# iacopo97/Multimodal-SAM-Adapter

Measured on AMD Instinct MI355X. Metric: images/sec encoder fwd @1024x1024 RGB+LiDAR ViT-L, higher is better.
Workload: dtype split-operand MFMA: fp16 hi + e5m2 cross terms (h8c / h8 planes, ViT / interaction / up-conv GEMMs) fp16 hi/lo pairs x3 (TwinConvNeXt: f3 planes) and bf16 hi/lo x3 (neck, head); attention blocks with the rel-pos terms fused: every contraction on one fp16 MFMA (q, k, v, P rounded to fp16) in the bloc

## Files before the change

include/mmsa.h:

```cpp
#ifndef MMSA_H
#define MMSA_H
#include <stddef.h>
#include <stdint.h>
#ifdef __cplusplus
extern "C" {
#endif

#ifdef MMSA_BUILDING_LIBRARY
typedef hipStream_t mmsa_stream_t;
#else
typedef void* mmsa_stream_t;
#endif

#include "mmsa_version.h"
int mmsa_version(void);
const char* mmsa_last_error(void);

int mmsa_debug_poison_lds(unsigned pattern, mmsa_stream_t stream);
int mmsa_event_create(void** ev);
int mmsa_event_record(void* ev, mmsa_stream_t stream);
int mmsa_event_elapsed_ms(void* start, void* stop, float* ms);
int mmsa_event_destroy(void* ev);

enum { MMSA_ACT_NONE = 0, MMSA_ACT_GELU = 1, MMSA_ACT_RELU = 2, MMSA_ACT_RELU6 = 3, MMSA_ACT_HSWISH = 4, MMSA_ACT_SIGMOID = 5 };
// ... 41 lines not shown
                            long strideW2, const float* b1, const float* b2, const float* gamma, float* x, long ldx, long strideX,
                            int M, int C, int batch, int max_grid, int fmt,
                            float* clamp_max , mmsa_stream_t stream);

int mmsa_split_planes(const float* src, long ld, int rows, int cols, int cols_pad, uint16_t* planes, int kind,
                      float* clamp_max , mmsa_stream_t stream);

int mmsa_attention(const float* qkv, long ldq, const float* qkv_bias, const float* rp, float* out, long ldo, int B,
                   int H, int W, int heads, int head_dim, int window_size, float scale, mmsa_stream_t stream);
int mmsa_attention_planes(const uint16_t* qkv_planes, long ldq, const uint16_t* bias_planes, const float* rp,
                          uint16_t* out_planes, long ldo, int B, int H, int W, int heads, int head_dim,
                          int window_size, float scale, int out_fmt ,
                          int v_fmt ,
                          float* max_abs_logit , mmsa_stream_t stream);

int mmsa_relpos_bias(const float* qkv, long ldq, const float* Rh, const float* Rw, float* rp, int B, int H, int W,
                     int heads, int head_dim, int window_size, mmsa_stream_t stream);
int mmsa_relpos_bias_planes(const uint16_t* qkv_planes, long ldq, const float* Rh, const float* Rw,
                            float* rp, int B, int H, int W, int heads, int head_dim, int window_size, mmsa_stream_t stream);

int mmsa_layernorm_rows(const float* x, long ldx, const float* w, const float* b, float eps, float* y, long ldy,
                        float* y2, long ldy2, uint16_t* y_planes, long ldp ,
                        int rows, int C, int map_mode, int map_H, int map_W, int group_rows, long w_gstride, long y_gcol,
                        int y_wrap, int plane_fmt , float* clamp_max ,
                        mmsa_stream_t stream);

int mmsa_colstats(const float* x, long ldx, long strideB, const float* wrow, int B, int HW, int C, double* out,
                  int out_is_zero , mmsa_stream_t stream);

int mmsa_ffrm_finalize(const double* stats, int B, int HW, int C, float mean_w, float mean_b, const float* Wc,
                       const float* gn_w, const float* gn_b, float* mean_o, float* rstd_o, float* mult_o,
                       float* scratch , mmsa_stream_t stream);
int mmsa_lnhw_apply(const float* x, long ldx, const float* mean, const float* rstd, const float* mult, const float* w,
                    const float* bias, float* y, long ldy, int B, int HW, int C, mmsa_stream_t stream);

int mmsa_dwconv_nhwc(const float* x, long ldx, long xstrideB, const float* w, const float* bias, float* y, long ldy,
                     long ystrideB, uint16_t* y_planes, long ldp, long pstrideB , int planes_fmt ,
                     int B, int H, int W, int C, int k, int act,
                     int imgs_per_group ,
                     float* rowstats ,
                     float* clamp_max , mmsa_stream_t stream);
int mmsa_gconv_nhwc(const float* x, long ldx, const float* w, const float* bias, float* y, long ldy, int B, int H,
                    int W, int G, int cin_g, int cout_g, int k, int act, mmsa_stream_t stream);
int mmsa_gfe_qkv_conv(const float* x, long ldx, const float* w, float* y, long ldy, int B, int H, int W, int G, int cin_g, int cout_g,
                      int* covered, mmsa_stream_t stream);
int mmsa_dwpair_gate(const float* x, long ldx, const float* w, float* y, long ldy, uint16_t* y_planes, long ldp, int B, int H,
                     int W, int C, mmsa_stream_t stream);
int mmsa_im2col_nchw(const float* x, int B, int Ctot, int c0, int Cin, int H, int W, int p, float* out, int Kpad,
                     mmsa_stream_t stream);

long mmsa_gram_tn_scratch_bytes(int B, int P, int c);
int mmsa_gram_tn(const float* X, long ldx, const float* Y, long ldy, long strideB, double* G , int B, int P, int c,
                 int nblk, void* scratch, long scratch_bytes, mmsa_stream_t stream);
int mmsa_chanattn_build(const double* G, const double* sq, long sq_strideB, const double* sk, long sk_strideB,
                        const float* temp, const float* Wp, uint16_t* planes , int B, int c, int cpad,
                        int heads, mmsa_stream_t stream);
int mmsa_gffm_build(const double* E, uint16_t* x_planes, uint16_t* y_planes , int B, int c,
                    int cpad, mmsa_stream_t stream);
int mmsa_gelu_gate(const float* x, long ldx, float* y, long ldy, long rows, int C, mmsa_stream_t stream);
int mmsa_pool_hw(const float* z, long ldz, float* out, long ldo, int B, int H, int W, int C, mmsa_stream_t stream);
int mmsa_ca_apply(const float* z, long ldz, const float* att, long lda, float* out, long ldo,
                  uint16_t* out_planes, long ldp , int B, int H, int W, int C, mmsa_stream_t stream);

int mmsa_tail_fuse(const float* cmap, long ldc, long cstrideB, const float* xtok, long ldx, const float* bn_scale,
                   const float* bn_shift, float* out, uint16_t* out_planes , long ldp,
                   int B, int Hc, int Wc, int Hx, int Wx, int C, mmsa_stream_t stream);

int mmsa_global_attention_planes(const uint16_t* qkv_planes, long ldq, const uint16_t* bias_planes, const uint16_t* relpos_planes,
                                 uint16_t* out_planes, long ldo, int B, int H, int W, int heads, int head_dim, float scale,
                                 int out_fmt , int v_fmt ,
                                 float* max_abs_logit , mmsa_stream_t stream);

int mmsa_window_attention_planes(const uint16_t* qkv_planes, long ldq, const uint16_t* bias_planes,
                                 const uint16_t* relpos_planes, const uint16_t* selector, uint16_t* out_planes, long ldo, int B, int H, int W,
                                 int heads, int head_dim, int window_size, float scale, int out_fmt ,
                                 int v_fmt , float* max_abs_logit , mmsa_stream_t stream);

int mmsa_nchw_to_planes(const float* src, long strideB, uint16_t* planes, long ldp, int B, int C, long HW,
                        mmsa_stream_t stream);
int mmsa_head_fuse(const float* z0, const float* z1, int H1, int W1, const float* z2, int H2, int W2, const float* z3,
                   int H3, int W3, long ld, const float* bn_scale, const float* bn_shift, uint16_t* planes, long ldp,
                   float* out32, long ldo, int B, int H, int W, int C, int act, mmsa_stream_t stream);
int mmsa_tokens_to_nchw(const float* src, long ld, float* dst, int B, long HW, int C, mmsa_stream_t stream);

int mmsa_bilinear_accum_nchw(const float* src, long src_strideB, int B, int C, int hs, int ws, float* dst, int Hd, int Wd, int y0, int x0,
                             int hc, int wc, float* count, int accumulate, mmsa_stream_t stream);
int mmsa_div_count_nchw(float* x, const float* count, int B, int C, long HW, mmsa_stream_t stream);
int mmsa_argmax_nchw(const float* x, unsigned char* out, int B, int C, long HW, mmsa_stream_t stream);
int mmsa_crop_batch_nchw(const float* src, int B, int C, int H, int W, const int* windows, int n, float* dst, int hc, int wc,
                         mmsa_stream_t stream);
int mmsa_slide_argmax(const float* logits, int n, int C, int hs, int ws, const int* windows, unsigned char* out, int B, int H, int W,
                      int hc, int wc, int* uncovered, mmsa_stream_t stream);
int mmsa_slide_argmax_resized(const float* logits, int n, int C, int hs, int ws, const int* windows, unsigned char* out, int B, int H, int W,
                              int hc, int wc, int Hd, int Wd, int Hcut, int Wcut, int* uncovered, mmsa_stream_t stream);

int mmsa_softmax_flip_accum_nchw(const float* logits, float* acc, int B, int C, int H, int W, int flip, int accumulate, int finish_div, mmsa_stream_t stream);
int mmsa_aug_argmax(const float* const* logits, const int* views, int A, int C, const int* windows, const int* windows_host, int total,
                    unsigned char* out, int B, int Ho, int Wo, int* uncovered, mmsa_stream_t stream);

int mmsa_argmax_max_nchw(const float* x, unsigned char* out, float* maxval, int B, int C, long HW, mmsa_stream_t stream);
int mmsa_slide_argmax_conf(const float* logits, int n, int C, int hs, int ws, const int* windows, unsigned char* out, float* conf, int B, int H, int W,
                           int hc, int wc, int* uncovered, mmsa_stream_t stream);
int mmsa_slide_argmax_resized_conf(const float* logits, int n, int C, int hs, int ws, const int* windows, unsigned char* out, float* conf, int B, int H,
                                   int W, int hc, int wc, int Hd, int Wd, int Hcut, int Wcut, int* uncovered, mmsa_stream_t stream);
int mmsa_aug_argmax_conf(const float* const* logits, const int* views, int A, int C, const int* windows, const int* windows_host, int total,
                         unsigned char* out, float* conf, int B, int Ho, int Wo, int* uncovered, mmsa_stream_t stream);

enum { MMSA_PRE_U8 = 0, MMSA_PRE_F32 = 1 };
int mmsa_preprocess_nhwc(const void* src0, int dtype0, const void* src1, int dtype1, int B, int Hs, int Ws, const float* mean,
                         const float* sinv, const int* div255, const int* swap, const float* pad_val, float* dst, int H, int W,
                         mmsa_stream_t stream);
int mmsa_preprocess_crops(const void* src0, int dtype0, const void* src1, int dtype1, int B, int Hs, int Ws, const float* mean,
                          const float* sinv, const int* div255, const int* swap, const float* pad_val, int H, int W, const int* windows,
                          int n, float* dst, int hc, int wc, mmsa_stream_t stream);
int mmsa_preprocess_resize_nhwc(const void* src0, int dtype0, const void* src1, int dtype1, int B, int Hs, int Ws, const float* mean,
                                const float* sinv, const int* div255, const int* swap, const float* pad_val, float* dst, int H, int W,
                                int Hr, int Wr, const int* xofs, const void* xcoef, const int* yofs, const void* ycoef, int fixed_point,
                                mmsa_stream_t stream);
int mmsa_preprocess_resize_crops(const void* src0, int dtype0, const void* src1, int dtype1, int B, int Hs, int Ws, const float* mean,
                                 const float* sinv, const int* div255, const int* swap, const float* pad_val, int H, int W, const int* windows,
                                 int n, float* dst, int hc, int wc, int Hr, int Wr, const int* xofs, const void* xcoef, const int* yofs,
                                 const void* ycoef, int fixed_point, mmsa_stream_t stream);

int mmsa_eval_confusion_u8(const unsigned char* pred, const unsigned char* label, int B, int H, int W, int Hl, int Wl, const unsigned char* lut,
                           int C, const int* ymap, const int* xmap, const int* slots, int n_slots, int64_t* counts, mmsa_stream_t stream);
int mmsa_slide_argmax_eval(const float* logits, int n, int C, int hs, int ws, const int* windows, unsigned char* out, int B, int H, int W,
                           int hc, int wc, int* uncovered, const unsigned char* label, int Hl, int Wl, const unsigned char* lut, const int* ymap,
                           const int* xmap, const int* slots, int n_slots, int64_t* counts, mmsa_stream_t stream);

int mmsa_eval_calibration(const unsigned char* pred, const float* conf, const unsigned char* label, int B, int H, int W, int Hl, int Wl,
                          const unsigned char* lut, int C, const int* ymap, const int* xmap, const int* slots, int n_slots, int bins, int64_t* cal,
                          mmsa_stream_t stream);

int mmsa_eval_selective(const unsigned char* pred, const float* conf, const unsigned char* label, int B, int H, int W, int Hl, int Wl,
                        const unsigned char* lut, int C, const int* ymap, const int* xmap, const int* slots, int n_slots, int bins, int64_t* counts,
                        mmsa_stream_t stream);
int mmsa_abstain_u8(const unsigned char* pred, const float* conf, long n, int bins, int min_bin, unsigned char* out, mmsa_stream_t stream);

int mmsa_slide_argmax_conf_t(const float* logits, int n, int C, int hs, int ws, const int* windows, unsigned char* out, float* conf, int B, int H, int W,
                             int hc, int wc, int* uncovered, float inv_temperature, mmsa_stream_t stream);
int mmsa_slide_argmax_resized_conf_t(const float* logits, int n, int C, int hs, int ws, const int* windows, unsigned char* out, float* conf, int B, int H,
                                     int W, int hc, int wc, int Hd, int Wd, int Hcut, int Wcut, int* uncovered, float inv_temperature, mmsa_stream_t stream);
int mmsa_softmax_flip_accum_nchw_t(const float* logits, float* acc, int B, int C, int H, int W, int flip, int accumulate, int finish_div,
                                   float inv_temperature, mmsa_stream_t stream);
int mmsa_temperature_sweep_nchw(const float* logits, const unsigned char* label, int B, int C, int H, int W, int Hl, int Wl, const unsigned char* lut,
                                const int* ymap, const int* xmap, const int* slots, int n_slots, const float* inv_temperatures, int J, int bins,
                                int64_t* sweep, mmsa_stream_t stream);

int mmsa_argmax_score_nchw(const float* prob, unsigned char* out, float* score, int B, int C, int H, int W, int kind, float inv_log_c, mmsa_stream_t stream);
int mmsa_slide_argmax_score(const float* logits, int n, int C, int hs, int ws, const int* windows, unsigned char* out, float* score, int B, int H, int W,
                            int hc, int wc, int* uncovered, int kind, float inv_temperature, float inv_log_c, mmsa_stream_t stream);
int mmsa_slide_argmax_resized_score(const float* logits, int n, int C, int hs, int ws, const int* windows, unsigned char* out, float* score, int B, int H,
                                    int W, int hc, int wc, int Hd, int Wd, int Hcut, int Wcut, int* uncovered, int kind, float inv_temperature,
                                    float inv_log_c, mmsa_stream_t stream);

int mmsa_slide_argmax_topk(const float* logits, int n, int C, int hs, int ws, const int* windows, unsigned char* classes, float* probs, int B, int H, int W,
                           int hc, int wc, int* uncovered, int K, float inv_temperature, mmsa_stream_t stream);
int mmsa_argmax_topk_nchw(const float* prob, const unsigned char* first, unsigned char* classes, float* probs, int B, int C, int H, int W, int K,
                          mmsa_stream_t stream);
int mmsa_eval_topk_u8(const unsigned char* classes, int K, const unsigned char* label, int B, int H, int W, int Hl, int Wl, const unsigned char* lut, int C,
                      const int* ymap, const int* xmap, const int* slots, int n_slots, int64_t* counts, mmsa_stream_t stream);

int mmsa_eval_boundary_u8(const unsigned char* pred, const unsigned char* label, int B, int H, int W, int Hl, int Wl, const unsigned char* lut, int C,
                          const int* ymap, const int* xmap, const int* slots, int n_slots, int radius, int border, int64_t* counts, mmsa_stream_t stream);

int mmsa_boundary_distance_u8(const unsigned char* src, int B, int Hs, int Ws, const unsigned char* lut, const int* ymap, const int* xmap, int H, int W,
// ... 76 lines not shown
```

multimodal-sam-adapter_amd/mmsa/head.py:

```python
import torch
import torch.nn as nn

from . import lib
from . import ops
from .params import Node, _attach


class SegformerHead(nn.Module):
    def __init__(self, interpolate_mode="bilinear", in_channels=None, channels=None, *, num_classes=None, dropout_ratio=0.1,
                 conv_cfg=None, norm_cfg=None, act_cfg=dict(type="ReLU"), in_index=-1, input_transform="multiple_select",
                 loss_decode=None, ignore_index=255, sampler=None, align_corners=False, init_cfg=None, **kwargs):
        super().__init__()
        if in_channels is None or channels is None or num_classes is None:
            raise TypeError("SegformerHead: in_channels, channels and num_classes are required")
        if not isinstance(in_channels, (list, tuple)) or not isinstance(in_index, (list, tuple)) or len(in_channels) != len(in_index):
            raise AssertionError("SegformerHead: in_channels and in_index must be lists of equal length")
        if not 1 <= len(in_channels) <= 4:
            raise NotImplementedError("mmsa SegformerHead: 1..4 input maps")
        if interpolate_mode != "bilinear" or align_corners:
            raise NotImplementedError("mmsa SegformerHead: only interpolate_mode='bilinear', align_corners=False (the reference configs)")
        if norm_cfg is None or norm_cfg.get("type") not in ("BN", "SyncBN"):
            raise NotImplementedError("mmsa SegformerHead: norm_cfg must be BN / SyncBN (eval: running-statistics affine)")
        if act_cfg is None or act_cfg.get("type") != "ReLU":
            raise NotImplementedError("mmsa SegformerHead: act_cfg must be ReLU")
        if channels % 8:
            raise NotImplementedError("mmsa SegformerHead: channels must be a multiple of 8")
        self.in_channels, self.in_index, self.channels = list(in_channels), list(in_index), channels
        self.num_classes, self.dropout_ratio, self.align_corners = num_classes, dropout_ratio, align_corners
        self.interpolate_mode, self.ignore_index, self.norm_cfg, self.act_cfg = interpolate_mode, ignore_index, norm_cfg, act_cfg
        n = len(in_channels)
        g = torch.Generator().manual_seed(0)

        def conv_w(co, ci):
            return torch.randn(co, ci, 1, 1, generator=g) * (2.0 / ci) ** 0.5

        def bn(prefix):
            _attach(self, prefix + ".weight", torch.ones(channels))
            _attach(self, prefix + ".bias", torch.zeros(channels))
            _attach(self, prefix + ".running_mean", torch.zeros(channels), buffer=True)
            _attach(self, prefix + ".running_var", torch.ones(channels), buffer=True)
            _attach(self, prefix + ".num_batches_tracked", torch.zeros((), dtype=torch.long), buffer=True)

        _attach(self, "conv_seg.weight", torch.randn(num_classes, channels, 1, 1, generator=g) * 0.01)
        _attach(self, "conv_seg.bias", torch.zeros(num_classes))
        self.add_module("convs", Node())
        for i, ci in enumerate(in_channels):
            _attach(self, f"convs.{i}.conv.weight", conv_w(channels, ci))
            bn(f"convs.{i}.bn")
        _attach(self, "fusion_conv.conv.weight", conv_w(channels, channels * n))
        bn("fusion_conv.bn")
        self._packed = None
        self._bufs = {}
        self.register_load_state_dict_post_hook(lambda m, _: m.invalidate())
        self.eval()

    def invalidate(self):
        self._packed = None

    def train(self, mode=True):
        if mode:
            raise NotImplementedError("mmsa: the MI355X decode head implements the inference forward path only")
        return super().train(False)

    def init_weights(self):
        pass

    def forward_test(self, inputs, img_metas=None, test_cfg=None):
        return self.forward(inputs)

    def forward_train(self, inputs, img_metas, gt_semantic_seg, train_cfg):
        raise NotImplementedError("mmsa: the MI355X decode head implements the inference forward path only (no losses)")

    @torch.no_grad()
    def _pack(self, dev):
        sd = {k: v.detach().to(dev, torch.float32) for k, v in self.state_dict().items() if v.dtype.is_floating_point}
        ch, n = self.channels, len(self.in_channels)

        def bn_affine(p):
            s = sd[p + ".weight"] / torch.sqrt(sd[p + ".running_var"] + 1e-5)
            return s.contiguous(), (sd[p + ".bias"] - sd[p + ".running_mean"] * s).contiguous()

        pk = {"branch": []}
        wf = sd["fusion_conv.conv.weight"].reshape(ch, ch * n)
        for i, ci in enumerate(self.in_channels):
            s, t = bn_affine(f"convs.{i}.bn")
            w = sd[f"convs.{i}.conv.weight"].reshape(ch, ci) * s[:, None]
            pk["branch"].append(dict(w=ops.split_planes(w.contiguous()), shift=t,
                                     wf=ops.split_planes(wf[:, ch * i:ch * (i + 1)].contiguous())))
        pk["fs"], pk["ft"] = bn_affine("fusion_conv.bn")
        ncp = ops.pad32(self.num_classes)
        wc = torch.zeros(ncp, ch, device=dev)
        wc[:self.num_classes] = sd["conv_seg.weight"].reshape(self.num_classes, ch)
        bc = torch.zeros(ncp, device=dev)
        bc[:self.num_classes] = sd["conv_seg.bias"]
        pk["wc"], pk["bc"], pk["ncp"] = ops.split_planes(wc), bc, ncp
        return pk

    def _buf(self, name, shape, dtype=torch.float32, dev=None):
        name = getattr(self, "buf_tag", "") + name
        t = self._bufs.get(name)
        if t is None or tuple(t.shape) != tuple(shape) or t.device != dev:
            t = torch.zeros(shape, dtype=dtype, device=dev)
            self._bufs[name] = t
        return t

    def _planes(self, name, rows, cols, dev):
        kp = ops.pad32(cols)
        return ops.Planes(self._buf(name, (rows, 2 * kp), torch.int16, dev), rows, cols, kp)

    @torch.no_grad()
    def forward(self, inputs, out=None):
        x0 = inputs[self.in_index[0]]
        if not x0.is_cuda:
            raise RuntimeError("mmsa SegformerHead: inputs must live on the GPU (there is no CPU path)")
        with torch.cuda.device(x0.device):
            return self._forward(inputs, out)

    def _forward(self, inputs, out=None):
        xs = [inputs[i] for i in self.in_index]
        x0 = xs[0]
        dev = x0.device
        if self._packed is None or self._packed["wc"].p.device != dev:
            self._packed = self._pack(dev)
        pk = self._packed
        B, _, H, W = x0.shape
        ch = self.channels
        zs = []
        for i, (x, ci) in enumerate(zip(xs, self.in_channels)):
            if x.dtype != torch.float32 or x.dim() != 4 or x.shape[0] != B or x.shape[1] != ci:
                raise RuntimeError(f"mmsa SegformerHead: input {i} must be fp32 [B={B}, {ci}, h, w], got {tuple(x.shape)} {x.dtype}")
            x = x.contiguous()
            h, w = x.shape[2:]
            rows = B * h * w
            xp = getattr(inputs[self.in_index[i]], "_mmsa_planes", None)
            if not isinstance(xp, ops.Planes) or xp.n != rows or xp.k != ci or xp.p.device != dev or not xp.live():
                xp = self._planes(f"x{i}", rows, ci, dev)
                lib.call("mmsa_nchw_to_planes", x.data_ptr(), ci * h * w, xp.p.data_ptr(), 2 * xp.kpad, B, ci, h * w, ops._stream())
            br = pk["branch"][i]
            yp = self._planes(f"y{i}", rows, ch, dev)
            ops.gemm(xp, br["w"], bias=br["shift"], act="relu", out_planes=yp)
            z = self._buf(f"z{i}", (rows, ch), dev=dev)
            ops.gemm(yp, br["wf"], z)
            zs.append((z, h, w))
        fp = self._planes("fused", B * H * W, ch, dev)
        lv = zs[1:] + [(None, 0, 0)] * (4 - len(zs))
        lib.call("mmsa_head_fuse", zs[0][0].data_ptr(),
                 lv[0][0].data_ptr() if lv[0][0] is not None else None, lv[0][1], lv[0][2],
                 lv[1][0].data_ptr() if lv[1][0] is not None else None, lv[1][1], lv[1][2],
                 lv[2][0].data_ptr() if lv[2][0] is not None else None, lv[2][1], lv[2][2],
                 ch, pk["fs"].data_ptr(), pk["ft"].data_ptr(), fp.p.data_ptr(), 2 * fp.kpad, None, 0, B, H, W, ch, ops.ACT["relu"],
                 ops._stream())
        lt = self._buf("logit_tokens", (B * H * W, pk["ncp"]), dev=dev)
        ops.gemm(fp, pk["wc"], lt, bias=pk["bc"])
        if out is None:
            out = torch.empty(B, self.num_classes, H, W, device=dev)
        elif (tuple(out.shape) != (B, self.num_classes, H, W) or out.dtype != torch.float32 or out.device != dev or not out.is_contiguous()):
            raise RuntimeError(f"mmsa SegformerHead: out must be a contiguous fp32 [{B}, {self.num_classes}, {H}, {W}] tensor on {dev}")
        lib.call("mmsa_tokens_to_nchw", lt.data_ptr(), pk["ncp"], out.data_ptr(), B, H * W, self.num_classes, ops._stream())
        return out
```

multimodal-sam-adapter_amd/mmsa/lib.py:

```python
import ctypes
import os
from ctypes import c_char_p, c_double, c_float, c_int, c_long, c_void_p, POINTER

_HERE = os.path.dirname(os.path.abspath(__file__))
LIB_PATH = os.environ.get("MMSA_LIB") or os.path.join(_HERE, "libmmsa_hip.so")

if not os.path.exists(LIB_PATH):
    raise RuntimeError(
        f"{LIB_PATH} not found: the MI355X HIP library is required (no CPU/PyTorch fallback exists). "
        "Build it with: python multimodal-sam-adapter_amd/build.py")

import torch

_lib = ctypes.CDLL(LIB_PATH)

P = c_void_p
I = c_int
L = c_long
F = c_float

_PAINT_TAIL = [P, I, P, I, I, I, I, I, P, P, I, I, c_double, c_double, c_double, c_double, P, P]
SIGNATURES = {
    "mmsa_version": [],
    "mmsa_last_error": [],
    "mmsa_debug_poison_lds": [ctypes.c_uint, P],
    "mmsa_event_create": [POINTER(c_void_p)],
    "mmsa_event_record": [P, P],
    "mmsa_event_elapsed_ms": [P, P, POINTER(c_float)],
    "mmsa_event_destroy": [P],
    "mmsa_ms_deform_attn_forward": [P, P, P, P, P, P, I, I, I, I, I, I, I, I, I, P],
    "mmsa_ms_deform_attn_backward": [P, P, P, P, P, P, P, P, P, I, I, I, I, I, I, I, I, I, P],
    "mmsa_msda_fused": [P, P, P, P, L, P, P, L, P, L, I, I, I, I, I, I, I, I, P, P],
    "mmsa_msda_fused_planes": [P, L, I, P, P, P, L, P, P, L, P, L, I, I, I, I, I, I, I, I, P, P],
    "mmsa_gemm_split3": [P, P, L, L, P, L, P, L, P, P, L, L, I, F, P, L, L, P, L, L, I, I, I, I, I, F, I, I, I, I, I, I, I, P, P, P, I, P, P],
    "mmsa_convnext_mlp_fused": [P, L, L, P, L, P, L, P, P, P, P, L, L, I, I, I, I, I, P, P],
    "mmsa_rowstats_finalize": [P, I, I, I, F, P, P],
    "mmsa_zero_bytes": [P, ctypes.c_size_t, P],
    "mmsa_split_planes": [P, L, I, I, I, P, I, P, P],
    "mmsa_attention": [P, L, P, P, P, L, I, I, I, I, I, I, F, P],
    "mmsa_attention_planes": [P, L, P, P, P, L, I, I, I, I, I, I, F, I, I, P, P],
    "mmsa_relpos_bias": [P, L, P, P, P, I, I, I, I, I, I, P],
    "mmsa_relpos_bias_planes": [P, L, P, P, P, I, I, I, I, I, I, P],
    "mmsa_layernorm_rows": [P, L, P, P, F, P, L, P, L, P, L, I, I, I, I, I, I, L, L, I, I, P, P],
    "mmsa_colstats": [P, L, L, P, I, I, I, P, I, P],
    "mmsa_ffrm_finalize": [P, I, I, I, F, F, P, P, P, P, P, P, P, P],
    "mmsa_lnhw_apply": [P, L, P, P, P, P, P, P, L, I, I, I, P],
    "mmsa_dwconv_nhwc": [P, L, L, P, P, P, L, L, P, L, L, I, I, I, I, I, I, I, I, P, P, P],
    "mmsa_dwpair_gate": [P, L, P, P, L, P, L, I, I, I, I, P],
    "mmsa_gconv_nhwc": [P, L, P, P, P, L, I, I, I, I, I, I, I, I, P],
    "mmsa_gfe_qkv_conv": [P, L, P, P, L, I, I, I, I, I, I, POINTER(c_int), P],
    "mmsa_im2col_nchw": [P, I, I, I, I, I, I, I, P, I, P],
    "mmsa_gram_tn": [P, L, P, L, L, P, I, I, I, I, P, L, P],
    "mmsa_gram_tn_scratch_bytes": [I, I, I],
    "mmsa_chanattn_build": [P, P, L, P, L, P, P, P, I, I, I, I, P],
    "mmsa_gffm_build": [P, P, P, I, I, I, P],
    "mmsa_gelu_gate": [P, L, P, L, L, I, P],
    "mmsa_pool_hw": [P, L, P, L, I, I, I, I, P],
    "mmsa_ca_apply": [P, L, P, L, P, L, P, L, I, I, I, I, P],
    "mmsa_tail_fuse": [P, L, L, P, L, P, P, P, P, L, I, I, I, I, I, I, P],
    "mmsa_global_attention_planes": [P, L, P, P, P, L, I, I, I, I, I, F, I, I, P, P],
    "mmsa_window_attention_planes": [P, L, P, P, P, P, L, I, I, I, I, I, I, F, I, I, P, P],
    "mmsa_nchw_to_planes": [P, L, P, L, I, I, L, P],
    "mmsa_head_fuse": [P, P, I, I, P, I, I, P, I, I, L, P, P, P, L, P, L, I, I, I, I, I, P],
    "mmsa_tokens_to_nchw": [P, L, P, I, L, I, P],
    "mmsa_bilinear_accum_nchw": [P, L, I, I, I, I, P, I, I, I, I, I, I, P, I, P],
    "mmsa_div_count_nchw": [P, P, I, I, L, P],
    "mmsa_argmax_nchw": [P, P, I, I, L, P],
    "mmsa_crop_batch_nchw": [P, I, I, I, I, P, I, P, I, I, P],
    "mmsa_slide_argmax": [P, I, I, I, I, P, P, I, I, I, I, I, P, P],
    "mmsa_slide_argmax_resized": [P, I, I, I, I, P, P, I, I, I, I, I, I, I, I, I, P, P],
    "mmsa_softmax_flip_accum_nchw": [P, P, I, I, I, I, I, I, I, P],
    "mmsa_aug_argmax": [P, P, I, I, P, P, I, P, I, I, I, P, P],
    "mmsa_argmax_max_nchw": [P, P, P, I, I, L, P],
    "mmsa_slide_argmax_conf": [P, I, I, I, I, P, P, P, I, I, I, I, I, P, P],
    "mmsa_slide_argmax_resized_conf": [P, I, I, I, I, P, P, P, I, I, I, I, I, I, I, I, I, P, P],
    "mmsa_aug_argmax_conf": [P, P, I, I, P, P, I, P, P, I, I, I, P, P],
    "mmsa_preprocess_nhwc": [P, I, P, I, I, I, I, P, P, P, P, P, P, I, I, P],
    "mmsa_preprocess_crops": [P, I, P, I, I, I, I, P, P, P, P, P, I, I, P, I, P, I, I, P],
    "mmsa_preprocess_resize_nhwc": [P, I, P, I, I, I, I, P, P, P, P, P, P, I, I, I, I, P, P, P, P, I, P],
    "mmsa_preprocess_resize_crops": [P, I, P, I, I, I, I, P, P, P, P, P, I, I, P, I, P, I, I, I, I, P, P, P, P, I, P],
    "mmsa_eval_confusion_u8": [P, P, I, I, I, I, I, P, I, P, P, P, I, P, P],
    "mmsa_eval_calibration": [P, P, P, I, I, I, I, I, P, I, P, P, P, I, I, P, P],
    "mmsa_eval_selective": [P, P, P, I, I, I, I, I, P, I, P, P, P, I, I, P, P],
    "mmsa_abstain_u8": [P, P, L, I, I, P, P],
    "mmsa_slide_argmax_conf_t": [P, I, I, I, I, P, P, P, I, I, I, I, I, P, F, P],
    "mmsa_slide_argmax_resized_conf_t": [P, I, I, I, I, P, P, P, I, I, I, I, I, I, I, I, I, P, F, P],
    "mmsa_softmax_flip_accum_nchw_t": [P, P, I, I, I, I, I, I, I, F, P],
    "mmsa_temperature_sweep_nchw": [P, P, I, I, I, I, I, I, P, P, P, P, I, P, I, I, P, P],
    "mmsa_argmax_score_nchw": [P, P, P, I, I, I, I, I, F, P],
    "mmsa_slide_argmax_score": [P, I, I, I, I, P, P, P, I, I, I, I, I, P, I, F, F, P],
    "mmsa_slide_argmax_resized_score": [P, I, I, I, I, P, P, P, I, I, I, I, I, I, I, I, I, P, I, F, F, P],
    "mmsa_slide_argmax_topk": [P, I, I, I, I, P, P, P, I, I, I, I, I, P, I, F, P],
    "mmsa_argmax_topk_nchw": [P, P, P, P, I, I, I, I, I, P],
    "mmsa_eval_topk_u8": [P, I, P, I, I, I, I, I, P, I, P, P, P, I, P, P],
    "mmsa_eval_boundary_u8": [P, P, I, I, I, I, I, P, I, P, P, P, I, I, I, P, P],
    "mmsa_boundary_distance_u8": [P, I, I, I, P, P, P, I, I, I, I, P, P, P],
    "mmsa_eval_boundary_d2": [P, P, I, I, I, I, I, P, I, P, P, P, I, P, P, I, P, P],
    "mmsa_eval_boundary_displacement": [P, P, I, I, I, I, I, P, I, P, P, P, I, P, P, I, P, P],
    "mmsa_components_u8": [P, I, I, I, P, P, P, I, I, I, P, P],
    "mmsa_component_area": [P, I, I, I, P, P],
    "mmsa_suppress_small_u8": [P, P, P, I, I, I, I, I, P, P],
    "mmsa_eval_segments": [P, P, I, I, I, I, I, P, I, P, P, P, I, P, P, I, P, P, P],
    "mmsa_segment_pairs": [P, P, I, I, P, I, P, P, P, P, I, I, I, P, P, L, P, P],
    "mmsa_eval_panoptic": [P, P, I, I, I, I, I, P, I, P, P, P, I, P, P, P, P, P, L, P, P, P],
    "mmsa_segment_table": [P, I, I, I, P, P, P, I, I, P, P, P, I, I, I, P, P, P, P, P],
    "mmsa_segment_table_block": [],
    "mmsa_select_segments_u8": [P, P, P, I, I, I, I, I, P, P],
    "mmsa_run_lengths_u8": [P, I, I, I, I, I, P, P, P, P, P],
    "mmsa_run_lengths_i32": [P, I, I, I, I, I, P, P, P, P, P],
    "mmsa_run_lengths_block": [I],
    "mmsa_run_decode_i32": [P, P, P, I, I, I, I, I, I, P, P],
    "mmsa_fill_nearest_u8": [P, I, I, I, P, I, I, P, P, P, P],
    "mmsa_majority_filter_u8": [P, I, I, I, P, I, I, I, P, P, P],
    "mmsa_vote_filter_u8": [P, I, I, I, P, I, I, I, P, I, I, I, P, P, P, P, P],
    "mmsa_slide_argmax_eval": [P, I, I, I, I, P, P, I, I, I, I, I, P, P, I, I, P, P, P, P, I, P, P],
    "mmsa_render_u8": [P, L, L, I, I, I, P, I, I, P, I, I, I, c_double, c_double, P, P],
    "mmsa_render_denorm_f32": [P, L, L, I, I, I, P, I, I, P, I, I, I, P, P, I, I, c_double, c_double, P, P],
    "mmsa_render_labels_u8": [P, L, L, P, I, I, I, I, I, P, I, P, P, I, I] + _PAINT_TAIL,
    "mmsa_render_values_f32": [P, P, L, L, I, I, I, I, I] + _PAINT_TAIL,
    "mmsa_render_band_u8": [P, L, L, P, I, I, I, I, I, P, I, P, P, I, I, I, I, I] + _PAINT_TAIL,
}
_RESTYPES = {"mmsa_last_error": c_char_p, "mmsa_gram_tn_scratch_bytes": c_long}

for _name, _args in SIGNATURES.items():
    _fn = getattr(_lib, _name)
    _fn.argtypes = _args
    _fn.restype = _RESTYPES.get(_name, c_int)


ABI_VERSION = 114
if _lib.mmsa_version() != ABI_VERSION:
    raise RuntimeError(f"{LIB_PATH}: ABI version {_lib.mmsa_version()} but mmsa/lib.py binds version {ABI_VERSION} (include/mmsa.h MMSA_ABI_VERSION): "
                       "rebuild with python multimodal-sam-adapter_amd/build.py")


def last_error() -> str:
    return _lib.mmsa_last_error().decode()


POISON_LDS = os.environ.get("MMSA_DEBUG_POISON_LDS") == "1"


def call(name, *args):
    if POISON_LDS and not name.startswith(("mmsa_event", "mmsa_debug")) and args:
        _lib.mmsa_debug_poison_lds(0x7FC07FC0, args[-1])
    rc = getattr(_lib, name)(*args)
    if rc != 0:
# ... 9 lines not shown
```

multimodal-sam-adapter_amd/mmsa/ops.py:

```python
import ctypes

import os

import torch

from . import lib

ACT = {"none": 0, "gelu": 1, "relu": 2, "relu6": 3, "hswish": 4, "sigmoid": 5}

GEMM_PROFILE = None
CLAMP_WATCH = None
GEMM_MAX_GRID = 0
GEMM_FLAVOUR = 0
GEMM_SHAPES = None


def _event():
    ev = ctypes.c_void_p()
    lib.call("mmsa_event_create", ctypes.byref(ev))
    return ev


def collect_gemm_profile(prof):
    flops, ms = 0.0, 0.0
# ... 504 lines not shown
    po, _, _, ldo = out.mat("out")
    lib.call("mmsa_global_attention_planes", pq, ldq, _chk(qkv_bias.p, torch.int16), _chk(relg.p, torch.int16), po, ldo,
             b, h, w, heads, hd, scale, out.fmt, _v_fmt(qkv, qkv_bias, heads * hd, fused=True, rel=relg), _guard(max_logit), _stream())
    return out


_SELECTORS = {}


def window_selector(ws, device, f16=False):
    key = (ws, str(device), f16)
    if key not in _SELECTORS:
        sel = torch.zeros(208, 32, dtype=torch.int16)
        j = torch.arange(min(ws * ws, 208))
        one = 0x3C00
        sel[j, j // ws] = one
        sel[j, 14 + j % ws] = one
        _SELECTORS[key] = sel.to(device)
    return _SELECTORS[key]


def window_attention(qkv, qkv_bias, relp, out, b, h, w, heads, hd, ws, scale, max_logit=None):
    if not 1 <= ws <= 14:
        raise RuntimeError(f"mmsa.window_attention: window_size {ws} not supported (1..14)")
    pq, _, _, ldq = qkv.mat("qkv")
    po, _, _, ldo = out.mat("out")
    vf = _v_fmt(qkv, qkv_bias, heads * hd, fused=True, rel=relp)
    lib.call("mmsa_window_attention_planes", pq, ldq, _chk(qkv_bias.p, torch.int16), _chk(relp.p, torch.int16),
             _chk(window_selector(ws, qkv.p.device, f16=vf == 2), torch.int16), po, ldo, b, h, w, heads, hd, ws, scale, out.fmt,
             vf, _guard(max_logit), _stream())
    return out


def colstats(x, stride_b, b, hw, out, wrow=None, out_is_zero=False):
    px, _, c, ldx = _mat(x, "x")
    lib.call("mmsa_colstats", px, ldx, stride_b, _chk(wrow), b, hw, c, _chk(out, torch.float64), int(out_is_zero), _stream())
    return out


def ffrm_finalize(stats, b, hw, c, mean_w, mean_b, wc, gn_w, gn_b, mean_o, rstd_o, mult_o, scratch):
    lib.call("mmsa_ffrm_finalize", _chk(stats, torch.float64), b, hw, c, mean_w, mean_b, _chk(wc), _chk(gn_w), _chk(gn_b),
             _chk(mean_o), _chk(rstd_o), _chk(mult_o), _chk(scratch), _stream())


def lnhw_apply(x, mean, rstd, mult, w, bias, out, b, hw):
    px, _, c, ldx = _mat(x, "x")
    po, _, _, ldo = _mat(out, "y")
    lib.call("mmsa_lnhw_apply", px, ldx, _chk(mean), _chk(rstd), _chk(mult), _chk(w), _chk(bias), po, ldo, b, hw, c, _stream())
    return out


def dwconv(x, w, bias, out, b, h, wd, k, act="none", xstride_b=None, ystride_b=None, out_planes=None, pstride_b=None,
           imgs_per_group=0, rowstats_out=None):
    px, _, c, ldx = _mat(x, "x")
    po, ldo = None, 0
    if out is not None:
        po, _, _, ldo = _mat(out, "y")
    pp, ldp = None, 0
    if out_planes is not None:
        pp, _, _, ldp = out_planes.mat("y planes")
    xs = h * wd * ldx if xstride_b is None else xstride_b
    ys = h * wd * ldo if ystride_b is None else ystride_b
    ps = h * wd * ldp if pstride_b is None else pstride_b
    lib.call("mmsa_dwconv_nhwc", px, ldx, xs, _chk(w), _chk(bias), po, ldo, ys, pp, ldp, ps, out_planes.fmt if out_planes is not None else FMT_B3,
             b, h, wd, c, k, ACT[act], imgs_per_group, _chk(rowstats_out), _clamp_ptr(), _stream())
    return out if out is not None else out_planes


def gconv(x, w, bias, out, b, h, wd, groups, cin_g, cout_g, k, act="none"):
    px, _, _, ldx = _mat(x, "x")
    po, _, _, ldo = _mat(out, "y")
    lib.call("mmsa_gconv_nhwc", px, ldx, _chk(w), _chk(bias), po, ldo, b, h, wd, groups, cin_g, cout_g, k, ACT[act], _stream())


def gfe_qkv(x, w12, out, b, h, wd, groups, cin_g, cout_g):
    px, _, _, ldx = _mat(x, "x")
    po, _, _, ldo = _mat(out, "y")
    covered = ctypes.c_int(0)
    lib.call("mmsa_gfe_qkv_conv", px, ldx, _chk(w12), po, ldo, b, h, wd, groups, cin_g, cout_g, ctypes.byref(covered), _stream())
    return bool(covered.value)
    return out


def dwpair_gate(x, w_tap, out, b, h, wd, c, out_planes=None):
    px, _, _, ldx = _mat(x, "x")
    po, ldo = (None, 0)
    if out is not None:
        po, _, _, ldo = _mat(out, "y")
    pp, ldp = (None, 0)
    if out_planes is not None:
        pp, _, _, ldp = out_planes.mat("y planes")
    lib.call("mmsa_dwpair_gate", px, ldx, _chk(w_tap), po, ldo, pp, ldp, b, h, wd, c, _stream())
    return out if out is not None else out_planes


def im2col_nchw(x, c0, cin, p, out):
    b, ctot, h, w = x.shape
    if not x.is_contiguous():
        raise RuntimeError("mmsa.im2col_nchw: input image must be contiguous NCHW")
    po, _, kpad, ld = _mat(out, "out")
    if ld != kpad:
        raise RuntimeError("mmsa.im2col_nchw: output must be dense")
    lib.call("mmsa_im2col_nchw", _chk(x), b, ctot, c0, cin, h, w, p, po, kpad, _stream())
    return out


def gram_tn_scratch_bytes(b, p, c):
    return int(lib.raw.mmsa_gram_tn_scratch_bytes(b, p, c))


def gram_tn(x, y, stride_b, g, b, p, nblk=1, scratch=None):
    px, _, c, ldx = _mat(x, "X")
    py, _, _, ldy = _mat(y, "Y")
    need = gram_tn_scratch_bytes(b, p, c)
    if scratch is None:
        scratch = torch.empty((need + 3) // 4, dtype=torch.float32, device=x.device)
    if not scratch.is_cuda or not scratch.is_contiguous():
        raise RuntimeError("gram_tn: scratch must be a contiguous device tensor")
    lib.call("mmsa_gram_tn", px, ldx, py, ldy, stride_b, _chk(g, torch.float64, "G"), b, p, c, nblk, scratch.data_ptr(),
             scratch.numel() * scratch.element_size(), _stream())
    return g


def chanattn_build(g, sq, sq_stride, sk, sk_stride, temp, wp, planes, b, c, heads):
    lib.call("mmsa_chanattn_build", _chk(g, torch.float64, "G"), sq, sq_stride, sk, sk_stride, _chk(temp), _chk(wp),
             planes.p.data_ptr(), b, c, planes.kpad, heads, _stream())


def gffm_build(e, px_, py_, b, c):
    lib.call("mmsa_gffm_build", _chk(e, torch.float64, "E"), px_.p.data_ptr(), py_.p.data_ptr(), b, c, px_.kpad, _stream())


def gelu_gate(x, out, c):
    px, rows, _, ldx = _mat(x, "x")
    po, _, _, ldo = _mat(out, "y")
    lib.call("mmsa_gelu_gate", px, ldx, po, ldo, rows, c, _stream())
    return out


def pool_hw(z, out, b, h, w):
    pz, _, c, ldz = _mat(z, "z")
    po, _, _, ldo = _mat(out, "out")
    lib.call("mmsa_pool_hw", pz, ldz, po, ldo, b, h, w, c, _stream())
    return out


def ca_apply(z, att, out, b, h, w, out_planes=None):
    pz, _, c, ldz = _mat(z, "z")
    pa, _, _, lda = _mat(att, "att")
    po, ldo = (None, 0)
    if out is not None:
        po, _, _, ldo = _mat(out, "out")
    pp, ldp = (None, 0)
    if out_planes is not None:
        pp, _, _, ldp = out_planes.mat("out planes")
    lib.call("mmsa_ca_apply", pz, ldz, pa, lda, po, ldo, pp, ldp, b, h, w, c, _stream())
    return out if out is not None else out_planes


def tail_fuse(cmap, cstride_b, xtok, bn_scale, bn_shift, out, b, hc, wc, hx, wx, out_planes=None):
    pc, _, c, ldc = _mat(cmap, "cmap")
    px, ldx = None, 0
    if xtok is not None:
        px, _, _, ldx = _mat(xtok, "xtok")
    pp, ldp = (out_planes.p.data_ptr(), 2 * out_planes.kpad) if out_planes is not None else (None, 0)
    lib.call("mmsa_tail_fuse", pc, ldc, cstride_b, px, ldx, _chk(bn_scale), _chk(bn_shift), _chk(out), pp, ldp, b, hc, wc, hx, wx, c, _stream())
# ... 2 lines not shown
```

Baseline: 67.59.

## Fuse head upsample-sum, BN-ReLU, classifier GEMM and NCHW store into one kernel

Adds a head_logits kernel that bilinearly samples and sums the multi-level head features, applies the BN affine and ReLU, and multiplies by the classifier weights with fp32 MFMA. It writes logits straight into the NCHW output. This replaces the head_fuse kernel, the plane-split GEMM and the tokens_to_nchw transpose, so the large fused-feature planes and logit-token buffers are never materialised in memory. The cost is recomputing the bilinear gathers per channel step and running fp32 MFMA instead of split-precision planes. The old path remains as a fallback for shapes the new kernel does not cover.

```diff
diff --git a/include/mmsa.h b/include/mmsa.h
--- a/include/mmsa.h
+++ b/include/mmsa.h
@@ -147,6 +147,9 @@
                    int H3, int W3, long ld, const float* bn_scale, const float* bn_shift, uint16_t* planes, long ldp,
                    float* out32, long ldo, int B, int H, int W, int C, int act, mmsa_stream_t stream);
 int mmsa_tokens_to_nchw(const float* src, long ld, float* dst, int B, long HW, int C, mmsa_stream_t stream);
+int mmsa_head_logits(const float* z0, const float* z1, int H1, int W1, const float* z2, int H2, int W2, const float* z3,
+                     int H3, int W3, long ld, const float* bn_scale, const float* bn_shift, const float* wc, const float* bc,
+                     float* out, int B, int H, int W, int C, int num_classes, int ncp, int act, int* covered, mmsa_stream_t stream);
 
 int mmsa_bilinear_accum_nchw(const float* src, long src_strideB, int B, int C, int hs, int ws, float* dst, int Hd, int Wd, int y0, int x0,
                              int hc, int wc, float* count, int accumulate, mmsa_stream_t stream);
diff --git a/multimodal-sam-adapter_amd/csrc/head_logits.hip b/multimodal-sam-adapter_amd/csrc/head_logits.hip
--- /dev/null
+++ b/multimodal-sam-adapter_amd/csrc/head_logits.hip
@@ -0,0 +1,199 @@
+#include "common.h"
+
+#define HL_MAX_WGS 512
+#define HL_WAVES 8
+
+struct HeadLogitLevels {
+  const float* z[3];
+  int H[3], W[3];
+  float rh[3], rw[3];
+};
+
+template <int NT, int NLV, int CMAX>
+__global__ __launch_bounds__(64 * HL_WAVES, (CMAX * NT * 64 + CMAX * 8 <= 80 * 1024) ? 2 : 1) void head_logits_kernel(
+    const float* __restrict__ z0, long ld, HeadLogitLevels lv, const float* __restrict__ bn_scale, const float* __restrict__ bn_shift,
+    const float* __restrict__ wc, const float* __restrict__ bc, float* __restrict__ out, int H, int W, int C, int num_classes, long npix, int ntiles,
+    int run, int relu) {
+  constexpr int NL = NLV > 0 ? NLV : 1;
+  __shared__ float4 wfrag[CMAX / 16 * NT * 64];
+  __shared__ float4 sbn[2 * (CMAX / 4)];
+  const int lane = threadIdx.x & 63, wave = threadIdx.x >> 6;
+  const int l15 = lane & 15, kk = lane >> 4;
+  const int steps = (C + 15) >> 4;
+
+  for (int i = threadIdx.x; i < steps * NT * 64; i += 64 * HL_WAVES) {
+    const int ln = i & 63, t = (i >> 6) % NT, j = (i >> 6) / NT;
+    const int c = 16 * j + 4 * (ln >> 4);
+    wfrag[i] = c < C ? *reinterpret_cast<const float4*>(wc + (long)(16 * t + (ln & 15)) * C + c) : make_float4(0.f, 0.f, 0.f, 0.f);
+  }
+  for (int i = threadIdx.x; i < 4 * steps; i += 64 * HL_WAVES) {
+    const bool in = 4 * i < C;
+    sbn[i] = in ? *reinterpret_cast<const float4*>(bn_scale + 4 * i) : make_float4(0.f, 0.f, 0.f, 0.f);
+    sbn[CMAX / 4 + i] = in ? *reinterpret_cast<const float4*>(bn_shift + 4 * i) : make_float4(0.f, 0.f, 0.f, 0.f);
+  }
+  __syncthreads();
+
+  const unsigned hw = (unsigned)H * (unsigned)W;
+  const int wg = (int)mmsa_xcd_order(blockIdx.x, gridDim.x);
+  const int t_end = min(ntiles, (wg + 1) * run);
+  for (int tile = wg * run + wave; tile < t_end; tile += HL_WAVES) {
+    const unsigned pg = (unsigned)min((long)tile * 16 + l15, npix - 1);
+    const int b = (int)(pg / hw);
+    const int rem = (int)(pg - (unsigned)b * hw);
+    const int h = rem / W, w = rem - h * W;
+    const float* p0 = z0 + (long)pg * ld;
+    const float* pl[NL];
+    unsigned dw[NL], dh[NL];
+    float w00[NL], w01[NL], w10[NL], w11[NL];
+#pragma unroll
+    for (int i = 0; i < NLV; ++i) {
+      float sh = ((float)h + 0.5f) * lv.rh[i] - 0.5f;
+      float sw = ((float)w + 0.5f) * lv.rw[i] - 0.5f;
+      sh = sh < 0.f ? 0.f : sh;
+      sw = sw < 0.f ? 0.f : sw;
+      const int h0 = min((int)sh, lv.H[i] - 1), w0 = min((int)sw, lv.W[i] - 1);
+      const float lh = sh - (float)h0, lw = sw - (float)w0;
+      pl[i] = lv.z[i] + (((long)b * lv.H[i] + h0) * lv.W[i] + w0) * ld;
+      dw[i] = w0 < lv.W[i] - 1 ? (unsigned)ld : 0u;
+      dh[i] = h0 < lv.H[i] - 1 ? (unsigned)lv.W[i] * (unsigned)ld : 0u;
+      w00[i] = (1.f - lh) * (1.f - lw); w01[i] = (1.f - lh) * lw; w10[i] = lh * (1.f - lw); w11[i] = lh * lw;
+    }
+    f32x4 acc[NT];
+#pragma unroll
+    for (int nt = 0; nt < NT; ++nt) {
+      const float bias = bc[16 * nt + l15];
+      acc[nt] = (f32x4){bias, bias, bias, bias};
+    }
+#pragma unroll 1
+    for (int j = 0; j < steps; ++j) {
+      const int c = 16 * j + 4 * kk;
+      const bool cin = c < C;
+      const int cl = cin ? c : 0;
+      const float4 a = *reinterpret_cast<const float4*>(p0 + cl);
+      float4 t[NL][4];
+#pragma unroll
+      for (int i = 0; i < NLV; ++i) {
+        const float* q = pl[i] + cl;
+        t[i][0] = *reinterpret_cast<const float4*>(q);
+        t[i][1] = *reinterpret_cast<const float4*>(q + dw[i]);
+        t[i][2] = *reinterpret_cast<const float4*>(q + dh[i]);
+        t[i][3] = *reinterpret_cast<const float4*>(q + dh[i] + dw[i]);
+      }
+      const float4 s = sbn[4 * j + kk], f = sbn[CMAX / 4 + 4 * j + kk];
+      float4 bf[NT];
+#pragma unroll
+      for (int nt = 0; nt < NT; ++nt) bf[nt] = wfrag[(j * NT + nt) * 64 + lane];
+      __builtin_amdgcn_sched_barrier(0);
+      float v[4] = {a.x, a.y, a.z, a.w};
+#pragma unroll
+      for (int i = 0; i < NLV; ++i) {
+        v[0] += w00[i] * t[i][0].x + w01[i] * t[i][1].x + w10[i] * t[i][2].x + w11[i] * t[i][3].x;
+        v[1] += w00[i] * t[i][0].y + w01[i] * t[i][1].y + w10[i] * t[i][2].y + w11[i] * t[i][3].y;
+        v[2] += w00[i] * t[i][0].z + w01[i] * t[i][1].z + w10[i] * t[i][2].z + w11[i] * t[i][3].z;
+        v[3] += w00[i] * t[i][0].w + w01[i] * t[i][1].w + w10[i] * t[i][2].w + w11[i] * t[i][3].w;
+      }
+      const float bs[4] = {s.x, s.y, s.z, s.w}, bt[4] = {f.x, f.y, f.z, f.w};
+#pragma unroll
+      for (int k = 0; k < 4; ++k) {
+        float x = v[k] * bs[k] + bt[k];
+        x = relu ? fmaxf(x, 0.f) : x;
+        v[k] = cin ? x : 0.f;
+      }
+#pragma unroll
+      for (int nt = 0; nt < NT; ++nt) {
+        acc[nt] = __builtin_amdgcn_mfma_f32_16x16x4f32(v[0], bf[nt].x, acc[nt], 0, 0, 0);
+        acc[nt] = __builtin_amdgcn_mfma_f32_16x16x4f32(v[1], bf[nt].y, acc[nt], 0, 0, 0);
+        acc[nt] = __builtin_amdgcn_mfma_f32_16x16x4f32(v[2], bf[nt].z, acc[nt], 0, 0, 0);
+        acc[nt] = __builtin_amdgcn_mfma_f32_16x16x4f32(v[3], bf[nt].w, acc[nt], 0, 0, 0);
+      }
+    }
+    const long q0 = (long)tile * 16 + 4 * kk;
+    if (q0 >= npix) continue;
+    const unsigned b0 = (unsigned)q0 / hw, r0 = (unsigned)q0 - b0 * hw;
+#pragma unroll
+    for (int nt = 0; nt < NT; ++nt) {
+      const int k = 16 * nt + l15;
+      if (k >= num_classes) continue;
+      float* o = out + ((long)b0 * num_classes + k) * hw + r0;
+      if (r0 + 3 < hw && (reinterpret_cast<uintptr_t>(o) & 15) == 0) {
+        *reinterpret_cast<float4*>(o) = make_float4(acc[nt][0], acc[nt][1], acc[nt][2], acc[nt][3]);
+      } else {
+#pragma unroll
+        for (int r = 0; r < 4; ++r) {
+          const long q = q0 + r;
+          if (q >= npix) break;
+          const unsigned bq = (unsigned)q / hw, rq = (unsigned)q - bq * hw;
+          out[((long)bq * num_classes + k) * hw + rq] = acc[nt][r];
+        }
+      }
+    }
+  }
+}
+
+template <int NT, int NLV, int CMAX>
+static void launch_head_logits(const float* z0, long ld, const HeadLogitLevels& lv, const float* bn_scale, const float* bn_shift, const float* wc,
+                               const float* bc, float* out, int H, int W, int C, int num_classes, long npix, int relu, hipStream_t stream) {
+  const int ntiles = cdiv(npix, 16);
+  const int nwg = min(HL_MAX_WGS, cdiv(ntiles, HL_WAVES));
+  const int run = cdiv(ntiles, nwg);
+  hipLaunchKernelGGL((head_logits_kernel<NT, NLV, CMAX>), dim3(nwg), dim3(64 * HL_WAVES), 0, stream, z0, ld, lv, bn_scale, bn_shift, wc, bc, out, H, W, C,
+                     num_classes, npix, ntiles, run, relu);
+}
+
+template <int NT, int CMAX>
+static void launch_head_logits_lv(int n, const float* z0, long ld, const HeadLogitLevels& lv, const float* bn_scale, const float* bn_shift,
+                                  const float* wc, const float* bc, float* out, int H, int W, int C, int num_classes, long npix, int relu,
+                                  hipStream_t stream) {
+  switch (n) {
+    case 0: launch_head_logits<NT, 0, CMAX>(z0, ld, lv, bn_scale, bn_shift, wc, bc, out, H, W, C, num_classes, npix, relu, stream); break;
+    case 1: launch_head_logits<NT, 1, CMAX>(z0, ld, lv, bn_scale, bn_shift, wc, bc, out, H, W, C, num_classes, npix, relu, stream); break;
+    case 2: launch_head_logits<NT, 2, CMAX>(z0, ld, lv, bn_scale, bn_shift, wc, bc, out, H, W, C, num_classes, npix, relu, stream); break;
+    default: launch_head_logits<NT, 3, CMAX>(z0, ld, lv, bn_scale, bn_shift, wc, bc, out, H, W, C, num_classes, npix, relu, stream); break;
+  }
+}
+
+extern "C" int mmsa_head_logits(const float* z0, const float* z1, int H1, int W1, const float* z2, int H2, int W2, const float* z3, int H3, int W3,
+                                long ld, const float* bn_scale, const float* bn_shift, const float* wc, const float* bc, float* out, int B, int H, int W,
+                                int C, int num_classes, int ncp, int act, int* covered, hipStream_t stream) {
+  MMSA_CHECK_ARG(z0 && bn_scale && bn_shift && wc && bc && out && covered, "head_logits: null pointer");
+  MMSA_CHECK_ARG(((((uintptr_t)bn_scale) | ((uintptr_t)bn_shift) | ((uintptr_t)z0) | ((uintptr_t)wc)) & 15) == 0,
+                 "head_logits: z0 / bn_scale / bn_shift / wc must be 16-byte aligned");
+  MMSA_CHECK_ARG((((uintptr_t)out) & 3) == 0, "head_logits: out must be 4-byte aligned");
+  MMSA_CHECK_ARG(B > 0 && H > 0 && W > 0 && C > 0 && C % 8 == 0, "head_logits: bad shape (C=%d must be a multiple of 8)", C);
+  MMSA_CHECK_ARG(ld >= C && ld % 4 == 0, "head_logits: row stride %ld", ld);
+  MMSA_CHECK_ARG(num_classes > 0 && ncp >= num_classes, "head_logits: %d classes in %d classifier rows", num_classes, ncp);
+  HeadLogitLevels lv;
+  int n = 0;
+  const float* zs[3] = {z1, z2, z3};
+  const int hs[3] = {H1, H2, H3}, wsz[3] = {W1, W2, W3};
+  for (int i = 0; i < 3; ++i) {
+    lv.z[i] = nullptr; lv.H[i] = lv.W[i] = 1; lv.rh[i] = lv.rw[i] = 1.f;
+  }
+  for (int i = 0; i < 3; ++i) {
+    if (!zs[i]) continue;
+    MMSA_CHECK_ARG(hs[i] > 0 && wsz[i] > 0, "head_logits: level %d has bad size", i + 1);
+    MMSA_CHECK_ARG((((uintptr_t)zs[i]) & 15) == 0, "head_logits: level %d must be 16-byte aligned", i + 1);
+    lv.z[n] = zs[i]; lv.H[n] = hs[i]; lv.W[n] = wsz[i];
+    lv.rh[n] = (float)hs[i] / (float)H;
+    lv.rw[n] = (float)wsz[i] / (float)W;
+    ++n;
+  }
+  const long npix = (long)B * H * W;
+  MMSA_CHECK_ARG(npix < (1L << 31), "head_logits: too many pixels for the 32-bit index arithmetic");
+  *covered = 0;
+  const int nt = num_classes <= 16 ? 1 : 2;
+  if (num_classes > 32 || ncp < 16 * nt || C > 1024 || (act != ACT_NONE && act != ACT_RELU)) return MMSA_OK;
+  for (int i = 0; i < n; ++i)
+    if ((long)lv.W[i] * ld >= (1L << 31)) return MMSA_OK;
+  const int relu = act == ACT_RELU;
+  if (C <= 512) {
+    if (nt == 1) launch_head_logits_lv<1, 512>(n, z0, ld, lv, bn_scale, bn_shift, wc, bc, out, H, W, C, num_classes, npix, relu, stream);
+    else launch_head_logits_lv<2, 512>(n, z0, ld, lv, bn_scale, bn_shift, wc, bc, out, H, W, C, num_classes, npix, relu, stream);
+  } else {
+    if (nt == 1) launch_head_logits_lv<1, 1024>(n, z0, ld, lv, bn_scale, bn_shift, wc, bc, out, H, W, C, num_classes, npix, relu, stream);
+    else launch_head_logits_lv<2, 1024>(n, z0, ld, lv, bn_scale, bn_shift, wc, bc, out, H, W, C, num_classes, npix, relu, stream);
+  }
+  MMSA_CHECK_LAUNCH("head_logits");
+  *covered = 1;
+  return MMSA_OK;
+}
diff --git a/multimodal-sam-adapter_amd/mmsa/head.py b/multimodal-sam-adapter_amd/mmsa/head.py
--- a/multimodal-sam-adapter_amd/mmsa/head.py
+++ b/multimodal-sam-adapter_amd/mmsa/head.py
@@ -7,6 +7,8 @@
 
 
 class SegformerHead(nn.Module):
+    fuse_logits = True
+
     def __init__(self, interpolate_mode="bilinear", in_channels=None, channels=None, *, num_classes=None, dropout_ratio=0.1,
                  conv_cfg=None, norm_cfg=None, act_cfg=dict(type="ReLU"), in_index=-1, input_transform="multiple_select",
                  loss_decode=None, ignore_index=255, sampler=None, align_corners=False, init_cfg=None, **kwargs):
@@ -94,6 +96,7 @@
         bc = torch.zeros(ncp, device=dev)
         bc[:self.num_classes] = sd["conv_seg.bias"]
         pk["wc"], pk["bc"], pk["ncp"] = ops.split_planes(wc), bc, ncp
+        pk["wc32"] = wc
         return pk
 
     def _buf(self, name, shape, dtype=torch.float32, dev=None):
@@ -142,6 +145,12 @@
             z = self._buf(f"z{i}", (rows, ch), dev=dev)
             ops.gemm(yp, br["wf"], z)
             zs.append((z, h, w))
+        if out is None:
+            out = torch.empty(B, self.num_classes, H, W, device=dev)
+        elif (tuple(out.shape) != (B, self.num_classes, H, W) or out.dtype != torch.float32 or out.device != dev or not out.is_contiguous()):
+            raise RuntimeError(f"mmsa SegformerHead: out must be a contiguous fp32 [{B}, {self.num_classes}, {H}, {W}] tensor on {dev}")
+        if self.fuse_logits and ops.head_logits(zs, pk["fs"], pk["ft"], pk["wc32"], pk["bc"], out, self.num_classes):
+            return out
         fp = self._planes("fused", B * H * W, ch, dev)
         lv = zs[1:] + [(None, 0, 0)] * (4 - len(zs))
         lib.call("mmsa_head_fuse", zs[0][0].data_ptr(),
@@ -152,9 +161,5 @@
                  ops._stream())
         lt = self._buf("logit_tokens", (B * H * W, pk["ncp"]), dev=dev)
         ops.gemm(fp, pk["wc"], lt, bias=pk["bc"])
-        if out is None:
-            out = torch.empty(B, self.num_classes, H, W, device=dev)
-        elif (tuple(out.shape) != (B, self.num_classes, H, W) or out.dtype != torch.float32 or out.device != dev or not out.is_contiguous()):
-            raise RuntimeError(f"mmsa SegformerHead: out must be a contiguous fp32 [{B}, {self.num_classes}, {H}, {W}] tensor on {dev}")
         lib.call("mmsa_tokens_to_nchw", lt.data_ptr(), pk["ncp"], out.data_ptr(), B, H * W, self.num_classes, ops._stream())
         return out
diff --git a/multimodal-sam-adapter_amd/mmsa/lib.py b/multimodal-sam-adapter_amd/mmsa/lib.py
--- a/multimodal-sam-adapter_amd/mmsa/lib.py
+++ b/multimodal-sam-adapter_amd/mmsa/lib.py
@@ -63,6 +63,7 @@
     "mmsa_nchw_to_planes": [P, L, P, L, I, I, L, P],
     "mmsa_head_fuse": [P, P, I, I, P, I, I, P, I, I, L, P, P, P, L, P, L, I, I, I, I, I, P],
     "mmsa_tokens_to_nchw": [P, L, P, I, L, I, P],
+    "mmsa_head_logits": [P, P, I, I, P, I, I, P, I, I, L, P, P, P, P, P, I, I, I, I, I, I, I, POINTER(c_int), P],
     "mmsa_bilinear_accum_nchw": [P, L, I, I, I, I, P, I, I, I, I, I, I, P, I, P],
     "mmsa_div_count_nchw": [P, P, I, I, L, P],
     "mmsa_argmax_nchw": [P, P, I, I, L, P],
diff --git a/multimodal-sam-adapter_amd/mmsa/ops.py b/multimodal-sam-adapter_amd/mmsa/ops.py
--- a/multimodal-sam-adapter_amd/mmsa/ops.py
+++ b/multimodal-sam-adapter_amd/mmsa/ops.py
@@ -610,6 +610,29 @@
     return out
 
 
+def head_logits(zs, bn_scale, bn_shift, wc, bc, out, num_classes, act="relu"):
+    pz, _, c, ld = _mat(zs[0][0], "z0")
+    b, _, h, wd = out.shape
+    if not out.is_contiguous() or out.shape[1] != num_classes or zs[0][0].shape[0] != b * zs[0][1] * zs[0][2] or (h, wd) != tuple(zs[0][1:]):
+        raise RuntimeError(f"mmsa.head_logits: out must be a contiguous [b, {num_classes}, {zs[0][1]}, {zs[0][2]}] tensor, got {tuple(out.shape)}")
+    if tuple(wc.shape) != (bc.shape[0], c) or not wc.is_contiguous():
+        raise RuntimeError(f"mmsa.head_logits: wc must be a contiguous [ncp, {c}] matrix with bc [ncp], got {tuple(wc.shape)} / {tuple(bc.shape)}")
+    lv = []
+    for i in range(1, 4):
+        if i < len(zs):
+            z, hl, wl = zs[i]
+            p, rows, cl, ldl = _mat(z, f"z{i}")
+            if (rows, cl, ldl) != (b * hl * wl, c, ld):
+                raise RuntimeError(f"mmsa.head_logits: z{i} must be [{b * hl * wl}, {c}] with row stride {ld}, got {tuple(z.shape)} stride {z.stride()}")
+            lv += [p, hl, wl]
+        else:
+            lv += [None, 0, 0]
+    covered = ctypes.c_int(0)
+    lib.call("mmsa_head_logits", pz, *lv, ld, _chk(bn_scale), _chk(bn_shift), _chk(wc), _chk(bc), _chk(out), b, h, wd, c, num_classes, bc.shape[0],
+             ACT[act], ctypes.byref(covered), _stream())
+    return bool(covered.value)
+
+
 def dwpair_gate(x, w_tap, out, b, h, wd, c, out_planes=None):
     px, _, _, ldx = _mat(x, "x")
     po, ldo = (None, 0)
```

After: 67.98, median of 6. Within noise of the previous version (+0.6%).
